# mapbox/robosat

Hardware: AMD Instinct MI355X
Metric: 512x512 tiles/sec train+predict, 1/2/4/8 MI355X; mIoU vs CPU ref (higher is better)
Workload: dtype f32; 1 GPU; rs predict ResNet50-UNet, bs=16 3x512x512 fp32 per GPU, 2 classes (BASELINE configs[1]); parallelism=tiles sharded over 1 rank(s), no collective

## Files before the change

### include/robosat_hip.h

```cpp
#ifndef ROBOSAT_HIP_H
#define ROBOSAT_HIP_H

#include <stdint.h>

#ifdef __cplusplus
extern "C" {
#endif

#define RS_EINVAL (-22)

typedef void* rs_stream_t;

typedef uint16_t rs_bf16;
#define RS_F32 0
#define RS_BF16 1

int rs_abi_version(void);

typedef struct rs_conv_desc {
  int32_t N;
  int32_t Hs, Ws;
  int32_t C1, C2;
  int32_t ups;
  int32_t kh, kw, stride, pad;
// ... 180 lines not shown
int rs_pack_s2_dgrad_phase_weight_dt(const float* w_krsc, void* out, int dtype, int Cout, int Cin, rs_stream_t stream);
int rs_conv2d_fwd_phase_dt(const rs_conv_desc* d, int dtype, const void* src1, const void* src2, const void* weight_phase,
                           const float* scale, const float* shift, const void* residual, const void* relu_mask, void* out,
                           rs_stream_t stream);

int rs_conv2d_splitk(const rs_conv_desc* d, int form, int* rowb);
int rs_conv2d_fwd_splitk(const rs_conv_desc* d, int form, const float* src1, const float* src2, const float* weight,
                         const float* scale, const float* shift, const float* residual, float* out, float* ws, int splits,
                         rs_stream_t stream);

int rs_conv2d_phase_wino_ok(const rs_conv_desc* d);
const char* rs_conv2d_phase_wino_name(const rs_conv_desc* d);
int rs_pack_wino_phase_weight(const float* w_phase, float* u, int Cout, int Cin, rs_stream_t stream);
int rs_conv2d_fwd_phase_wino(const rs_conv_desc* d, const float* src1, const float* src2, const float* u, float* out,
                             rs_stream_t stream);
int rs_conv2d_dgrad_phase_wino_ok(const rs_conv_desc* d);
const char* rs_conv2d_dgrad_phase_wino_name(const rs_conv_desc* d);
int rs_pack_wino_dgrad_weight(const float* wd4x4, float* u, int Cin, int Cout, rs_stream_t stream);
int rs_conv2d_dgrad_phase_wino(const rs_conv_desc* d, const float* dz, const float* u, float* out, const float* mask, float* out2,
                               const float* mask2, int csplit, rs_stream_t stream);

int rs_conv2d_wino33_ok(const rs_conv_desc* d);
const char* rs_conv2d_wino33_name(const rs_conv_desc* d);
int rs_pack_wino33_weight(const float* w_krsc, float* u, int Cout, int Cin, rs_stream_t stream);
int rs_conv2d_fwd_wino33(const rs_conv_desc* d, const float* src, const float* u, const float* scale, const float* shift, float* out,
                         rs_stream_t stream);
int rs_conv2d_wino33_head_ok(const rs_conv_desc* d, int C);
const char* rs_conv2d_wino33_head_name(void);
int rs_conv2d_fwd_wino33_head(const rs_conv_desc* d, const float* src, const float* u, const float* scale, const float* shift,
                              const float* final_w, const float* final_b, int C, int mode, const double* anchors, int overlap,
// ... 170 lines not shown
```

### robosat_amd/_lib.py

```python

import ctypes
import os
from ctypes import POINTER, c_char_p, c_float, c_int, c_int32, c_long, c_void_p

import torch

_HERE = os.path.dirname(os.path.abspath(__file__))
LIB_PATH = os.environ.get("ROBOSAT_HIP_LIB") or os.path.join(_HERE, "librobosat_hip.so")

RS_EINVAL = -22
ABI_VERSION = 24
RS_F32, RS_BF16 = 0, 1
RS_TTA_IN_U8, RS_TTA_IN_F32 = 0, 1
RS_TTA_PROBS, RS_TTA_QUANTIZE, RS_TTA_ARGMAX = 0, 1, 2


class ConvDesc(ctypes.Structure):

    _fields_ = [
        ("N", c_int32), ("Hs", c_int32), ("Ws", c_int32), ("C1", c_int32), ("C2", c_int32), ("ups", c_int32),
        ("kh", c_int32), ("kw", c_int32), ("stride", c_int32), ("pad", c_int32), ("Ho", c_int32), ("Wo", c_int32),
        ("Cout", c_int32), ("relu", c_int32), ("stem", c_int32),
    ]

# ... 78 lines not shown
    "rs_bn_bwd_dt": (c_int, [P, P, P, P, P, P, P, P, P, P, c_int, c_long, c_int, P, P]),
    "rs_upsample2x_bwd_dt": (c_int, [P, P, P, P, P, c_int, c_int, c_int, c_int, c_int, c_int, c_int, P]),
    "rs_conv2d_bnstats_rows": (c_long, [POINTER(ConvDesc)]),
    "rs_conv2d_bnstats_rows_dt": (c_long, [POINTER(ConvDesc), c_int]),
    "rs_conv2d_fwd_bnstats_dt": (c_int, [POINTER(ConvDesc), c_int, P, P, P, P, P, P]),
    "rs_bn_finalize_stats": (c_int, [P, c_long, c_long, c_int, c_float, c_float, P, P, P, P, P, P, P, P, P, P, P]),
    "rs_pack_phase_weight_dt": (c_int, [P, P, c_int, c_int, c_int, P]),
    "rs_pack_s2_dgrad_phase_weight_dt": (c_int, [P, P, c_int, c_int, c_int, P]),
    "rs_conv2d_fwd_phase_dt": (c_int, [POINTER(ConvDesc), c_int, P, P, P, P, P, P, P, P, P]),
    "rs_conv2d_splitk": (c_int, [POINTER(ConvDesc), c_int, POINTER(c_int)]),
    "rs_conv2d_fwd_splitk": (c_int, [POINTER(ConvDesc), c_int, P, P, P, P, P, P, P, P, c_int, P]),
    "rs_conv2d_phase_wino_ok": (c_int, [POINTER(ConvDesc)]),
    "rs_conv2d_phase_wino_name": (c_char_p, [POINTER(ConvDesc)]),
    "rs_pack_wino_phase_weight": (c_int, [P, P, c_int, c_int, P]),
    "rs_conv2d_fwd_phase_wino": (c_int, [POINTER(ConvDesc), P, P, P, P, P]),
    "rs_conv2d_dgrad_phase_wino_ok": (c_int, [POINTER(ConvDesc)]),
    "rs_conv2d_dgrad_phase_wino_name": (c_char_p, [POINTER(ConvDesc)]),
    "rs_pack_wino_dgrad_weight": (c_int, [P, P, c_int, c_int, P]),
    "rs_conv2d_dgrad_phase_wino": (c_int, [POINTER(ConvDesc), P, P, P, P, P, P, c_int, P]),
    "rs_conv2d_wino33_ok": (c_int, [POINTER(ConvDesc)]),
    "rs_conv2d_wino33_name": (c_char_p, [POINTER(ConvDesc)]),
    "rs_pack_wino33_weight": (c_int, [P, P, c_int, c_int, P]),
    "rs_conv2d_fwd_wino33": (c_int, [POINTER(ConvDesc), P, P, P, P, P, P]),
    "rs_conv2d_wino33_head_ok": (c_int, [POINTER(ConvDesc), c_int]),
    "rs_conv2d_wino33_head_name": (c_char_p, []),
    "rs_conv2d_fwd_wino33_head": (c_int, [POINTER(ConvDesc), P, P, P, P, P, P, c_int, c_int, P, c_int, P, P, P]),
    "rs_bottleneck_tail_f32": (c_int, [P, P, P, P, P, P, P, P, P, P, c_long, c_int, c_int, c_int, P]),
    "rs_conv1x1_wave_f32": (c_int, [P, P, P, P, P, c_int, P, c_long, c_int, c_int, P]),
    "rs_conv2d_wino33_stats_rows": (c_long, [POINTER(ConvDesc)]),
    "rs_conv2d_fwd_wino33_stats": (c_int, [POINTER(ConvDesc), P, P, P, P, P]),
# ... 107 lines not shown
```

### robosat_amd/csrc/common.h

```cpp
#pragma once
#include <hip/hip_runtime.h>
#include <stdint.h>

#include "../../include/robosat_hip.h"

typedef float f32x4 __attribute__((ext_vector_type(4)));
typedef float f32x16 __attribute__((ext_vector_type(16)));
typedef __bf16 bf16_t;
typedef __bf16 bf16x4 __attribute__((ext_vector_type(4)));
typedef __bf16 bf16x8 __attribute__((ext_vector_type(8)));
typedef unsigned int u32x2 __attribute__((ext_vector_type(2)));
typedef unsigned int u32x4 __attribute__((ext_vector_type(4)));
typedef short s16x4 __attribute__((ext_vector_type(4)));
typedef short s16x8 __attribute__((ext_vector_type(8)));

__device__ __forceinline__ f32x4 rs_ld4(const float* p) { return *reinterpret_cast<const f32x4*>(p); }
__device__ __forceinline__ f32x4 rs_ld4(const bf16_t* p) {
  return __builtin_convertvector(*reinterpret_cast<const bf16x4*>(p), f32x4);
}
__device__ __forceinline__ void rs_st4(float* p, f32x4 v) { *reinterpret_cast<f32x4*>(p) = v; }
__device__ __forceinline__ void rs_st4(bf16_t* p, f32x4 v) {
  *reinterpret_cast<bf16x4*>(p) = __builtin_convertvector(v, bf16x4);
}
__device__ __forceinline__ float rs_ld1(const float* p) { return *p; }
// ... 166 lines not shown
  int halo_ko = 0;
  int wgrad_f32_phase = 1;
  int wgrad_f32_dma = -1;
  int wgrad_f32_blocks = 2048;
  int wgrad_f32_wino = 1;
  int wgrad_f32_wino_blocks = 1024;
  int wgrad_f32_wino33 = 1;
  int wgrad_f32_wino33_blocks = 256;
  int wgrad_blocks = 96;
  int wgrad_blocks_phase = 1536;
  int wgrad_phase4 = 1;
  int wgrad_blocks_phase4 = 256;
  int wgrad_ring = 3;
  int lovasz_xcd = 1;
  int wino_wide = 1;
  int grow_fused = 0;
};
__attribute__((visibility("hidden"))) RsKnobs& rs_knobs();

__attribute__((visibility("hidden"))) int rs_wgrad_thin_plan(const rs_conv_desc* d, int* blocks, int* slices);
__attribute__((visibility("hidden"))) int rs_wgrad_thin_launch(const rs_conv_desc* d, const void* dy, const void* src,
                                                               float* partial, void* stream);

__attribute__((visibility("hidden"))) int rs_conv_thin_bf16_launch(int mode, const void* src, const void* wgt, const void* mask,
                                                                   void* out, int N, int Hs, int Ws, int relu, void* stream);

__attribute__((visibility("hidden"))) long rs_reduce_scratch_floats(long n, int splits);
__attribute__((visibility("hidden"))) int rs_reduce_splits(const float* ws, float* out, long n, int splits, float* scratch,
                                                           void* stream);

// ... 6 lines not shown
```

### robosat_amd/csrc/conv_wino_f32.hip

```cpp
#define RS_CONV_INSTANTIATE
#include "conv_igemm_dma_kernel.h"

namespace {

struct WinoArgs {
  const float* src1;
  const float* src2;
  const float* u;
  float* out;
  int N, Hs, Ws, C1, C2, Cout;
  int TY, TX;
  int BBY, BBX;
  int nsub;
  int ncb;
  int relu;
  float* out2;
  const float* mask1;
  const float* mask2;
  int csplit;
};

template <int PB>
struct WinoGeom {
  static constexpr int HW = 2 * PB + 1;
  static constexpr int PITCH = HW;
  static constexpr int HALF = PB + 1;
  static constexpr int SBROWS = (HW * PITCH + 7) / 8 * 8;
};

template <int PB>
__device__ __forceinline__ int wino_lane_tile(int l) {
  if constexpr (PB == 8) return ((l & 1) << 1) | (((l >> 1) & 1) << 2) | ((l >> 2) & 1) | (l & 8);
  return ((l & 1) << 1) | (((l >> 1) & 1) << 3) | ((l >> 2) & 1) | (((l >> 3) & 1) << 2);
}
typedef float f32x2 __attribute__((ext_vector_type(2)));
__device__ __forceinline__ f32x2 pk_sub(f32x2 a, f32x2 b) {
  f32x2 d;
  asm("v_pk_add_f32 %0, %1, %2 neg_lo:[0,1] neg_hi:[0,1]" : "=v"(d) : "v"(a), "v"(b));
  return d;
}
__device__ __forceinline__ int wino_lane_now() {
  int l;
  asm volatile("v_mbcnt_lo_u32_b32 %0, -1, 0\n\tv_mbcnt_hi_u32_b32 %0, -1, %0" : "=v"(l));
  return l;
}
__device__ __forceinline__ int wino_swz(int row) { return (row ^ (row >> 1)) & 3; }

template <int PB, int TG, int CG, int NM = 2, bool DG = false>
__global__ __launch_bounds__(512, 1) void conv_wino_f32_kernel(const WinoArgs p) {
  using G = WinoGeom<PB>;
  constexpr int NW = TG * CG;
  static_assert(NW == 8, "8 waves");
  constexpr int BMT = 16 * TG, BN = 16 * NM * CG;
  constexpr int SB = BMT / (PB * PB);
  static_assert(SB * PB * PB == BMT, "whole sub-blocks per block");
  constexpr int AROWS = SB * G::SBROWS;
  constexpr int IA = (AROWS + 15) / 16, IB = 9 * BN / 16;
  constexpr int AROWS_PAD = IA * 16;
  constexpr int JA = (IA + NW - 1) / NW, JB = (IB + NW - 1) / NW;
  constexpr int NI = JA + JB;
  constexpr int STAGE = (AROWS_PAD + 9 * BN) * 64;
  constexpr int KC = 16;

  constexpr int NTR = (AROWS_PAD + 64 * NW - 1) / (64 * NW);
  __shared__ __attribute__((aligned(16))) unsigned char smem[2 * STAGE + 2 * AROWS_PAD * 4 + NTR * 64 * NW * 4];
  int* tabs = reinterpret_cast<int*>(smem + 2 * STAGE);

  int* trows = tabs + 2 * AROWS_PAD;
  const int tid = threadIdx.x, lane = tid & 63;
  const int wave = __builtin_amdgcn_readfirstlane(tid >> 6);
  const int tg = wave % TG, cg = wave / TG;
  const int per_img = p.BBY * p.BBX;
  const int Cin = p.C1 + p.C2;
  const int nk = Cin / KC;
  const int ntiles = ((p.nsub + SB - 1) / SB) * p.ncb * (DG ? 1 : 4);
  const int first = rs_xcd_remap(blockIdx.x, gridDim.x);
  const int nitems = (ntiles - first + (int)gridDim.x - 1) / (int)gridDim.x * (DG ? 4 : 1);
  const unsigned int lds0 = __builtin_amdgcn_readfirstlane(rs_lds_addr(smem));
  const long img1 = (long)p.Hs * p.Ws * p.C1 * (DG ? 4 : 1), img2 = (long)p.Hs * p.Ws * p.C2;

  constexpr int SBS = SB <= 2 ? SB : 1;
  struct Item {
    int py, px, nblk, nfirst, sub0;
    int n[SBS], y0[SBS], x0[SBS];
    bool live[SBS];
  };
  const int uni_first = __builtin_amdgcn_readfirstlane(first), uni_grid = __builtin_amdgcn_readfirstlane((int)gridDim.x);
  const int d_step = DG ? uni_grid : uni_grid >> 2, d_parstep = DG ? 1 : uni_grid & 3;
  int d_par = DG ? 0 : uni_first & 3;
  int d_mblk = (DG ? uni_first : uni_first >> 2) / p.ncb, d_nblk = (DG ? uni_first : uni_first >> 2) - d_mblk * p.ncb;
  const int dq = d_step / p.ncb, dr = d_step - dq * p.ncb;
  auto decode_next = [&](Item& s) __attribute__((always_inline)) {
    s.py = d_par >> 1;
    s.px = d_par & 1;
    if (!DG || d_par == 0) {
      s.nblk = d_nblk;
      const int sub0 = s.sub0 = d_mblk * SB;
      int n = __builtin_amdgcn_readfirstlane(sub0 / per_img);
      const int r2 = sub0 - n * per_img;
      int bby = __builtin_amdgcn_readfirstlane(r2 / p.BBX);
      int bbx = r2 - bby * p.BBX;
      s.nfirst = n;
#pragma unroll
      for (int sb = 0; sb < SBS; ++sb) {
        s.live[sb] = sub0 + sb < p.nsub;
        s.n[sb] = n;
        s.y0[sb] = 2 * bby * PB - 1;
        s.x0[sb] = 2 * bbx * PB - 1;
        if (++bbx == p.BBX) {
          bbx = 0;
          if (++bby == p.BBY) {
            bby = 0;
            ++n;
          }
        }
      }
    }
    d_par += d_parstep;
    const int carry = d_par >> 2;
    d_par &= 3;
    if (!DG || carry) {
      d_mblk += dq;
      d_nblk += dr + (DG ? 0 : carry);
      if (d_nblk >= p.ncb) {
        d_nblk -= p.ncb;
        ++d_mblk;
      }
    }
  };
  Item cur, nxt;
  decode_next(cur);
  nxt = cur;
  auto sub_block = [&](const Item& s, int sb, int& n, int& y0, int& x0, bool& live) __attribute__((always_inline)) {
    if constexpr (SB <= 2) {
      const bool one = SB > 1 && sb > 0;
      n = one ? s.n[SBS - 1] : s.n[0];
      y0 = one ? s.y0[SBS - 1] : s.y0[0];
      x0 = one ? s.x0[SBS - 1] : s.x0[0];
// ... 1 lines not shown
    } else {
      const int sub = s.sub0 + sb;
      n = sub / per_img;
      const int r2 = sub - n * per_img, bby = r2 / p.BBX, bbx = r2 - bby * p.BBX;
      y0 = 2 * bby * PB - 1;
      x0 = 2 * bbx * PB - 1;
      live = sub < p.nsub;
    }
  };

#pragma unroll
  for (int e = 0; e < NTR; ++e) {
    const int rho = tid + 64 * NW * e;
    const int sb = rho / G::SBROWS, rem = rho - sb * G::SBROWS;
    const int hy = rem / G::PITCH, xs = rem - hy * G::PITCH;
    const int hx = xs < G::HALF ? 2 * xs : 2 * (xs - G::HALF) + 1;
    trows[rho] = ((rho < AROWS && hy < G::HW) ? hy << 16 : -(1 << 28)) | (hx << 8) | sb;
  }
  auto build_table = [&](const Item& s, int seq) __attribute__((always_inline)) {
    int* tab = tabs + (seq & 1) * AROWS_PAD;
    const int tnow = 64 * wave + wino_lane_now();
#pragma unroll
    for (int e = 0; e < NTR; ++e) {
      const int rho = tnow + 64 * NW * e;
      if (rho < AROWS_PAD) {
        int n, y0, x0;
        bool live;
        const int row = trows[rho];
        sub_block(s, row & 255, n, y0, x0, live);
        const int y = y0 + s.py + (row >> 16), x = x0 + s.px + ((row >> 8) & 255);
        const bool in = live && (unsigned)y < (unsigned)p.Hs && (unsigned)x < (unsigned)p.Ws;
        const int v = DG ? ((n - s.nfirst) * 2 * p.Hs + 2 * y + 1 - s.py) * (2 * p.Ws) + 2 * x + 1 - s.px
                         : ((n - s.nfirst) * p.Hs + y) * p.Ws + x;
        tab[rho] = in ? v : -1;
      }
    }
    rs_lds_writes_done();
  };

  const int ra = lane >> 2, pp = lane & 3;
  static_assert(128 % BN == 0, "a wave's filter pieces: the same cout, whole positions apart");
  int doff[JA], doffu;
  {
    const int w = 16 * wave + ra, xi = w / BN, co = w - xi * BN;
    doffu = ((xi * p.Cout + co) * Cin) * 4 + ((pp ^ wino_swz(w)) & 3) * 16;
  }
  const int ustep = (128 / BN) * p.Cout * Cin * 4;
  int f_seq = 0, f_kc = 0, f_g = 0;
  int f_nb = 0, f_nfirst = 0;
  __amdgpu_buffer_rsrc_t rsrcs = rs_dma_rsrc<kDmaClamp>(p.src1, 0), rsrcu = rsrcs;
  auto fetch_item = [&](const Item& s) __attribute__((always_inline)) {
    f_nfirst = s.nfirst;
    f_nb = s.nblk * BN * Cin * 4;
    rsrcu = rs_dma_rsrc<kDmaClamp>(p.u + (long)(2 * s.py + s.px) * 9 * p.Cout * Cin, (long)9 * p.Cout * Cin * 4);
  };
  auto set_source = [&](bool src_first) __attribute__((always_inline)) {
    const int cb = (src_first ? p.C1 : p.C2) * 4;
    rsrcs = rs_dma_rsrc<kDmaClamp>(src_first ? p.src1 + f_nfirst * img1 : p.src2 + f_nfirst * img2,
                                   (long)(p.N - f_nfirst) * (src_first ? img1 : img2) * 4);
    const int* tab = tabs + (f_seq & 1) * AROWS_PAD;
    int pix[JA];
#pragma unroll
    for (int j = 0; j < JA; ++j) {
      const int ii = wave + NW * j;
      pix[j] = tab[16 * (ii < IA ? ii : IA - 1) + ra];
    }
#pragma unroll
    for (int j = 0; j < JA; ++j) {
      const int ii = wave + NW * j;
// ... 4 lines not shown
  auto fetch_chunk = [&](auto interleave, bool past) __attribute__((always_inline)) {
    const int c0 = f_kc * KC;
    const bool src_first = c0 < p.C1;
    if (!past) {
      if (f_kc == 0) fetch_item(nxt);
      if (c0 == 0 || c0 == p.C1) set_source(src_first);
    }
    const unsigned int fL = lds0 + (f_g & 1) * STAGE;
    const int fsa = __builtin_amdgcn_readfirstlane((src_first ? c0 : c0 - p.C1) * 4), fsu = __builtin_amdgcn_readfirstlane(c0 * 4 + f_nb);
    interleave([&](int j) __attribute__((always_inline)) {
      if (j < JA) {
        const int ii = wave + NW * j;
        if (j < JA - 1 || JA * NW == IA || ii < IA) rs_dma16(rsrcs, fL + ii * 1024, doff[j], fsa);
      } else {
        const int fi = wave + NW * (j - JA);
        if (j < NI - 1 || JB * NW == IB || fi < IB) rs_dma16(rsrcu, fL + (IA + fi) * 1024, doffu, fsu + (j - JA) * ustep);
      }
    });
    ++f_g;
    if (!past && ++f_kc == nk) {
      f_kc = 0;
      ++f_seq;
    }
  };

  const int l15 = lane & 15, pc = lane >> 4;
  const int t = 16 * tg + wino_lane_tile<PB>(l15);
  const int tsb = 16 * tg / (PB * PB), tq = t - tsb * (PB * PB);
  const int tty = tq / PB, ttx = tq - tty * PB;
  int addrA[3][3];
  {
    const int rho0 = tsb * G::SBROWS + 2 * tty * G::PITCH + ttx;
#pragma unroll
    for (int r = 0; r < 3; ++r)
#pragma unroll
      for (int c = 0; c < 3; ++c) {
        const int rho = rho0 + r * G::PITCH + (c == 0 ? 0 : (c == 1 ? G::HALF : 1));
        addrA[r][c] = rho * 64 + ((pc ^ wino_swz(rho)) & 3) * 16;
      }
  }
  const int addrB = AROWS_PAD * 64 + (16 * NM * cg + l15) * 64 + ((pc ^ wino_swz(l15)) & 3) * 16;

  build_table(cur, 0);
  __syncthreads();
  fetch_chunk([&](auto issue) __attribute__((always_inline)) {
#pragma unroll
    for (int j = 0; j < NI; ++j) issue(j);
  }, false);
  const int total = nitems * nk;
  const int Ho = 2 * p.Hs, Wo = 2 * p.Ws;

#ifdef RS_WINO_TAIL2
  constexpr int TAIL = NM >= 4 ? 1 : RS_WINO_TAIL2;
#else
  constexpr int TAIL = NM >= 4 ? 1 : PB == 4 ? 2 : (DG || TG == 8) ? 0 : 1;
#endif
  static_assert(TAIL >= 0 && TAIL <= 2, "positions behind the barrier");
  constexpr int NMMA = 36 * NM, NHEAD = (9 - TAIL) * 4 * NM, NT = TAIL * 4 * NM;
  constexpr int PSTEP = 2 * NMMA / 3 / NI >= 1 ? 2 * NMMA / 3 / NI : 1;
  static_assert((NI - 1) * PSTEP < NHEAD, "the DMA pieces go out in the chunk's head");
  f32x4 V[9], Bq[9][NM];
  auto chunk_head = [&](const unsigned char* L, f32x4(&Vn)[9], f32x4(&B0)[NM], auto tail, auto nt) __attribute__((always_inline)) {
    constexpr int N = decltype(nt)::value, LEAD = N / 2;
    f32x4 P[3][3];
#pragma unroll
    for (int r = 0; r < 3; ++r)
#pragma unroll
      for (int c = 0; c < 3; ++c) P[r][c] = *reinterpret_cast<const f32x4*>(L + addrA[r][c]);
    __builtin_amdgcn_sched_barrier(0);
#pragma unroll
// ... 106 lines not shown
            const int a = a0 + u, b = b0 + v;
            if (a >= p.Hs || b >= p.Ws) continue;
            const long o = ((long)(e_n * p.Hs + a) * p.Ws + b) * ostride + ocol;
#pragma unroll
            for (int m = 0; m < NM; ++m) {
              f32x4 y = (acc[u * 3 + v][m] + acc[u * 3 + v + 1][m]) + (acc[(u + 1) * 3 + v][m] + acc[(u + 1) * 3 + v + 1][m]);
              if (mb) {
                const f32x4 z = *reinterpret_cast<const f32x4*>(mb + o + 16 * m);
#pragma unroll
                for (int e = 0; e < 4; ++e) y[e] = z[e] > 0.f ? y[e] : 0.f;
              }
              *reinterpret_cast<f32x4*>(ob + o + 16 * m) = y;
            }
          }
      }
    } else if (e_live) {
      float* obase = p.out + cur.nblk * BN + 16 * NM * cg + 4 * e_pc;
#pragma unroll
      for (int u = 0; u < 2; ++u)
#pragma unroll
        for (int v = 0; v < 2; ++v) {
          const int a = a0 + u, b = b0 + v;
          if (a >= p.Hs || b >= p.Ws) continue;
          float* o = obase + ((long)(e_n * Ho + 2 * a + cur.py) * Wo + 2 * b + cur.px) * p.Cout;
#pragma unroll
          for (int m = 0; m < NM; ++m) {
            f32x4 y = (acc[u * 3 + v][m] + acc[u * 3 + v + 1][m]) + (acc[(u + 1) * 3 + v][m] + acc[(u + 1) * 3 + v + 1][m]);
            if (p.relu) {
#pragma unroll
              for (int e = 0; e < 4; ++e) y[e] = fmaxf(y[e], 0.f);
// ... 26 lines not shown
  const int co = (int)(i % Cout);
  const long r = i / Cout;
  const int ci = (int)(r % Cin), ph = (int)(r / Cin), py = ph >> 1, px = ph & 1;
  const float* g = wd + (long)ci * 16 * Cout + co;
  const float g00 = g[(long)(py * 4 + px) * Cout], g01 = g[(long)(py * 4 + 2 + px) * Cout];
  const float g10 = g[(long)((2 + py) * 4 + px) * Cout], g11 = g[(long)((2 + py) * 4 + 2 + px) * Cout];
  const float v[9] = {g00, g00 + g01, g01, g00 + g10, (g00 + g01) + (g10 + g11), g01 + g11, g10, g10 + g11, g11};
#pragma unroll
  for (int x = 0; x < 9; ++x) u[(((long)ph * 9 + x) * Cin + ci) * Cout + co] = v[x];
}

bool wino_wide() {
  return rs_knobs().wino_wide != 0;
}

struct WinoPlan {
  int pb, wgn;
  int sb;
  bool worth;
  bool wide;
};

bool wino_plan(const rs_conv_desc* d, WinoPlan* pl) {
  if (!d || d->N <= 0 || d->Hs <= 0 || d->Ws <= 0 || d->C1 <= 0 || (d->C1 % 16) || d->C2 < 0 || (d->C2 % 16) || d->Cout <= 0 ||
      (d->Cout % 32))
    return false;
  if (!(d->ups == 1 && d->kh == 3 && d->kw == 3 && d->stride == 1 && d->pad == 1 && d->Ho == 2 * d->Hs && d->Wo == 2 * d->Ws)) return false;
  const int ty = (d->Hs + 1) / 2, tx = (d->Ws + 1) / 2;
  if (ty < 4 || tx < 4) return false;
  pl->pb = (ty >= 8 && tx >= 8) ? 8 : 4;
  pl->wgn = (d->Cout % 64 == 0) ? 2 : 1;
  pl->sb = 16 * (8 / pl->wgn) / (pl->pb * pl->pb);
  if (d->C1 + d->C2 < 32) return false;
  const long cmax = d->C1 > d->C2 ? d->C1 : d->C2;
  if ((long)(pl->sb + 1) * d->Hs * d->Ws * cmax * 4 >= (1L << 31)) return false;
  if ((long)9 * d->Cout * (d->C1 + d->C2) * 4 >= (1L << 31)) return false;
  if ((long)d->N * d->Ho * d->Wo >= (1L << 31)) return false;
  pl->worth = pl->pb == 8;
  pl->wide = false;
  if (pl->pb == 8 && pl->wgn == 2 && wino_wide()) {
    const long nsub = (long)d->N * rs_cdiv(ty, 8) * rs_cdiv(tx, 8);
    pl->wide = (nsub + 1) / 2 * (d->Cout / 64) * 4 >= 2L * rs_cu_count();
    if (pl->wide) pl->sb = 2;
  }
  return true;
}

}

extern "C" int rs_conv2d_phase_wino_ok(const rs_conv_desc* d) {
  WinoPlan pl;
  if (!wino_plan(d, &pl)) return 0;
  return pl.worth ? 1 : 2;
}

extern "C" const char* rs_conv2d_phase_wino_name(const rs_conv_desc* d) {
  WinoPlan pl;
  if (!wino_plan(d, &pl)) return "";
  if (pl.pb == 8) return pl.wide ? "conv_wino_f32<phase,p8,128x64>" : (pl.wgn == 2 ? "conv_wino_f32<phase,p8,64x64>" : "conv_wino_f32<phase,p8,128x32>");
  return pl.wgn == 2 ? "conv_wino_f32<phase,p4,64x64>" : "conv_wino_f32<phase,p4,128x32>";
}

extern "C" int rs_pack_wino_phase_weight(const float* w_phase, float* u, int Cout, int Cin, rs_stream_t stream) {
  if (!w_phase || !u || Cout <= 0 || Cin <= 0) return RS_EINVAL;
  const long total = 4L * Cout * Cin;
  pack_wino_phase_weight_kernel<<<rs_cdiv(total, 256), 256, 0, (hipStream_t)stream>>>(w_phase, u, Cout, Cin, total);
  return RS_LAUNCH_RESULT();
}

extern "C" int rs_conv2d_fwd_phase_wino(const rs_conv_desc* d, const float* src1, const float* src2, const float* u, float* out,
                                        rs_stream_t stream) {
  WinoPlan pl;
  if (!wino_plan(d, &pl) || !src1 || !u || !out || (d->C2 > 0 && !src2)) return RS_EINVAL;
  WinoArgs a;
  a.src1 = src1;
  a.src2 = src2;
  a.u = u;
  a.out = out;
  a.N = d->N;
  a.Hs = d->Hs;
  a.Ws = d->Ws;
  a.C1 = d->C1;
  a.C2 = d->C2;
  a.Cout = d->Cout;
  a.TY = (d->Hs + 1) / 2;
  a.TX = (d->Ws + 1) / 2;
  a.BBY = rs_cdiv(a.TY, pl.pb);
  a.BBX = rs_cdiv(a.TX, pl.pb);
  a.nsub = d->N * a.BBY * a.BBX;
  a.ncb = d->Cout / (32 * pl.wgn);
  a.relu = d->relu;
  a.out2 = nullptr;
  a.mask1 = a.mask2 = nullptr;
  a.csplit = 0;
  const long items = (long)rs_cdiv(a.nsub, pl.sb) * a.ncb * 4;
  if (items >= (1L << 31)) return RS_EINVAL;
  const int grid = (int)(items < rs_cu_count() ? items : rs_cu_count());
  hipStream_t s = (hipStream_t)stream;
  if (pl.wide) conv_wino_f32_kernel<8, 8, 1, 4><<<grid, 512, 0, s>>>(a);
  else if (pl.pb == 8 && pl.wgn == 2) conv_wino_f32_kernel<8, 4, 2><<<grid, 512, 0, s>>>(a);
  else if (pl.pb == 8) conv_wino_f32_kernel<8, 8, 1><<<grid, 512, 0, s>>>(a);
  else if (pl.wgn == 2) conv_wino_f32_kernel<4, 4, 2><<<grid, 512, 0, s>>>(a);
  else conv_wino_f32_kernel<4, 8, 1><<<grid, 512, 0, s>>>(a);
  return RS_LAUNCH_RESULT();
}

namespace {
bool wino_dgrad_plan(const rs_conv_desc* d, rs_conv_desc* g, WinoPlan* pl) {
  if (!d || d->C1 <= 0 || d->C2 < 0 || d->Cout <= 0) return false;
  *g = *d;
  g->C1 = d->Cout;
  g->C2 = 0;
  g->Cout = d->C1 + d->C2;
  if (!wino_plan(g, pl) || !pl->worth) return false;
  if ((long)(pl->sb + 1) * 4 * d->Hs * d->Ws * g->C1 * 4 >= (1L << 31)) return false;
  if (g->Cout % 64) return false;
  return true;
}
}

extern "C" int rs_conv2d_dgrad_phase_wino_ok(const rs_conv_desc* d) {
  rs_conv_desc g;
  WinoPlan pl;
  return wino_dgrad_plan(d, &g, &pl) ? 1 : 0;
}

extern "C" const char* rs_conv2d_dgrad_phase_wino_name(const rs_conv_desc* d) {
  rs_conv_desc g;
  WinoPlan pl;
  if (!wino_dgrad_plan(d, &g, &pl)) return "";
  return pl.wide ? "conv_wino_f32<dgrad4x4,p8,128x64>" : "conv_wino_f32<dgrad4x4,p8,64x64>";
// ... 22 lines not shown
  a.mask2 = mask2;
  a.csplit = csplit;
  a.N = d->N;
  a.Hs = d->Hs;
  a.Ws = d->Ws;
  a.C1 = g.C1;
  a.C2 = 0;
  a.Cout = g.Cout;
  a.TY = (d->Hs + 1) / 2;
  a.TX = (d->Ws + 1) / 2;
  a.BBY = rs_cdiv(a.TY, pl.pb);
  a.BBX = rs_cdiv(a.TX, pl.pb);
  a.nsub = d->N * a.BBY * a.BBX;
  a.ncb = g.Cout / 64;
  a.relu = 0;
  bool wide = false;
  if (wino_wide()) wide = (long)((a.nsub + 1) / 2) * a.ncb >= 2L * rs_cu_count();
  const int sb = wide ? 2 : 1;
  const long items = (long)rs_cdiv(a.nsub, sb) * a.ncb;
  if (items >= (1L << 29)) return RS_EINVAL;
  const int grid = (int)(items < rs_cu_count() ? items : rs_cu_count());
  hipStream_t s = (hipStream_t)stream;
  if (wide) conv_wino_f32_kernel<8, 8, 1, 4, true><<<grid, 512, 0, s>>>(a);
  else conv_wino_f32_kernel<8, 4, 2, 2, true><<<grid, 512, 0, s>>>(a);
  return RS_LAUNCH_RESULT();
}
```

### robosat_amd/csrc/knobs.hip

```cpp
#include <stdio.h>
#include <stdlib.h>
#include <string.h>

#include "common.h"

namespace {

struct Entry {
  const char* name;
  const char* env;
  int RsKnobs::*field;
  int lo, hi;
};

bool in_range(const Entry& e, int v) {
  if (v < e.lo || v > e.hi) return false;
  if (e.field == &RsKnobs::conv_rowb) return v == 0 || v == 64 || v == 128;
  return true;
}

const Entry kEntries[] = {
    {"conv_tile", "RS_CONV_TILE", &RsKnobs::conv_tile, -1, 9},
    {"conv_rowb", "RS_CONV_ROWB", &RsKnobs::conv_rowb, 0, 128},
    {"conv_big", "RS_CONV_BIG", &RsKnobs::conv_big, 0, 1},
// ... 8 lines not shown
    {"halo_ko", "RS_HALO_KO", &RsKnobs::halo_ko, 0, 4},
    {"wgrad_f32_phase", "RS_WGRAD_F32_PHASE", &RsKnobs::wgrad_f32_phase, 0, 1},
    {"wgrad_f32_dma", "RS_WGRAD_F32_DMA", &RsKnobs::wgrad_f32_dma, -1, 1},
    {"wgrad_f32_blocks", "RS_WGRAD_F32_BLOCKS", &RsKnobs::wgrad_f32_blocks, 1, 1048576},
    {"wgrad_f32_wino", "RS_WGRAD_F32_WINO", &RsKnobs::wgrad_f32_wino, 0, 1},
    {"wgrad_f32_wino_blocks", "RS_WGRAD_F32_WINO_BLOCKS", &RsKnobs::wgrad_f32_wino_blocks, 1, 1048576},
    {"wgrad_f32_wino33", "RS_WGRAD_F32_WINO33", &RsKnobs::wgrad_f32_wino33, 0, 1},
    {"wgrad_f32_wino33_blocks", "RS_WGRAD_F32_WINO33_BLOCKS", &RsKnobs::wgrad_f32_wino33_blocks, 1, 1048576},
    {"wgrad_blocks", "RS_WGRAD_BLOCKS", &RsKnobs::wgrad_blocks, 1, 1048576},
    {"wgrad_blocks_phase", "RS_WGRAD_BLOCKS_PHASE", &RsKnobs::wgrad_blocks_phase, 1, 1048576},
    {"wgrad_phase4", "RS_WGRAD_PHASE4", &RsKnobs::wgrad_phase4, 0, 1},
    {"wgrad_blocks_phase4", "RS_WGRAD_BLOCKS_PHASE4", &RsKnobs::wgrad_blocks_phase4, 1, 1048576},
    {"wgrad_ring", "RS_WGRAD_RING", &RsKnobs::wgrad_ring, 2, 7},
    {"lovasz_xcd", "RS_LOVASZ_XCD", &RsKnobs::lovasz_xcd, 0, 1},
    {"wino_wide", "ROBOSAT_WINO_WIDE", &RsKnobs::wino_wide, 0, 1},
    {"grow_fused", "RS_GROW_FUSED", &RsKnobs::grow_fused, 0, 16},
};

}

RsKnobs& rs_knobs() {
  static RsKnobs k = [] {
    RsKnobs v;
    for (const Entry& e : kEntries)
      if (const char* s = getenv(e.env)) {
        const int x = atoi(s);
        if (in_range(e, x)) v.*(e.field) = x;
        else fprintf(stderr, "robosat_hip: %s=%s is outside [%d, %d]: ignored, the rule stays\n", e.env, s, e.lo, e.hi);
      }
    return v;
// ... 25 lines not shown
```

### robosat_amd/ops.py

```python

import ctypes
import os

import torch

from . import _lib
from ._lib import RS_BF16, RS_F32, ConvDesc, check

BF16 = torch.bfloat16


def _dt(t):

    dtype = getattr(t, "dtype", t)
    if dtype == torch.float32:
        return RS_F32
    if dtype == torch.bfloat16:
        return RS_BF16
    raise TypeError("robosat_amd: activations are fp32 or bf16, got {}".format(dtype))


def _esize(t):

    return 2 if getattr(t, "dtype", t) == BF16 else 4
# ... 338 lines not shown
    if src1.dtype != torch.float32 or not (force or switch("ROBOSAT_WINOGRAD")):
        return False
    d = _phase_desc(*src1.shape, 0 if src2 is None else src2.shape[3], cout)
    rc = _lib.lib().rs_conv2d_phase_wino_ok(ctypes.byref(d))
    return rc != 0 if force else rc == 1


def pack_wino_phase_weight(weight_phase):

    _, cout, _, _, cin = weight_phase.shape
    u = torch.empty((4, 9, cout, cin), device=weight_phase.device, dtype=torch.float32)
    _call("rs_pack_wino_phase_weight", _dev(weight_phase, "w_phase"), _dev(u, "u"), cout, cin, _stream())
    return u


def conv2d_phase_wino(src1, u, src2=None, relu=False):

    n, hs, ws, c1 = src1.shape
    c2 = 0 if src2 is None else src2.shape[3]
    cout = u.shape[2]
    assert tuple(u.shape) == (4, 9, cout, c1 + c2)
    if src2 is not None and tuple(src2.shape[:3]) != (n, hs, ws):
        raise RuntimeError("Sizes of tensors must match except in dimension 1: skip {} vs decoder {}".format(
            tuple(src1.shape[:3]), tuple(src2.shape[:3])))
    d = _phase_desc(n, hs, ws, c1, c2, cout, relu)
    out = torch.empty((n, 2 * hs, 2 * ws, cout), device=src1.device, dtype=torch.float32)
    ev = _start()
    _call("rs_conv2d_fwd_phase_wino", ctypes.byref(d), _dev(src1, "src1"), _dev(src2, "src2"), _dev(u, "u"), _dev(out, "out"), _stream())
    if ev:
        _stop(ev)
        name = _lib.lib().rs_conv2d_phase_wino_name(ctypes.byref(d)).decode()
        _record(ev, name, conv_flops(d), _shape(d), conv_bytes(d, 4), conv_flops(d) * 0.25)
    return out


def wino_dgrad_ok(n, hs, ws, c1, c2, cout):

    if not switch("ROBOSAT_WINO_DGRAD"):
        return False
    return _lib.lib().rs_conv2d_dgrad_phase_wino_ok(ctypes.byref(_phase_desc(n, hs, ws, c1, c2, cout))) == 1


def pack_wino_dgrad_weight(wd4x4):
# ... 1709 lines not shown
```

### robosat_amd/unet.py

```python

import math
import os
import warnings

import torch
import torch.nn as nn

from . import ops

_RESNET50_FILE = "resnet50-19c8e357.pth"


class _Conv(nn.Module):

    def __init__(self, cin, cout, k, stride=1, padding=0, bias=False, init="default"):
        super().__init__()
        self.cin, self.cout, self.k, self.stride, self.padding = cin, cout, k, stride, padding
        w = torch.empty(cout, cin, k, k).contiguous(memory_format=torch.channels_last)
        fan_in, fan_out = cin * k * k, cout * k * k
        if init == "resnet":
            nn.init.normal_(w, 0.0, math.sqrt(2.0 / fan_out))
        else:
            nn.init.uniform_(w, -1.0 / math.sqrt(fan_in), 1.0 / math.sqrt(fan_in))
        self.weight = nn.Parameter(w)
# ... 176 lines not shown
    def __init__(self, num_in, num_out):
        super().__init__()
        self.block = ConvRelu(num_in, num_out)


def conv3x3_eval(conv, x, dt, scale=None, shift=None):

    if dt == torch.float32 and conv.stride == 1 and ops.wino33_ok(x, conv.cout):
        return ops.conv2d_wino33(x, conv.wino33(), scale=scale, shift=shift, relu=True)
    return ops.conv2d(x, conv.krsc(dt), stride=conv.stride, pad=1, scale=scale, shift=shift, relu=True)


def decoder_block(conv, skip, prev, dt):

    if dt == torch.float32 and ops.wino_ok(skip, prev, conv.cout):
        return ops.conv2d_phase_wino(skip, conv.phase_wino(), src2=prev, relu=True)
    return ops.conv2d_phase(skip, conv.phase(dt), src2=prev, relu=True)


def _find_pretrained():
    cands = [os.environ.get("ROBOSAT_RESNET50_WEIGHTS")]
    home = os.environ.get("TORCH_HOME", os.path.join(os.path.expanduser("~"), ".cache", "torch"))
    cands += [os.path.join(home, "checkpoints", _RESNET50_FILE), os.path.join(home, "hub", "checkpoints", _RESNET50_FILE)]
    for c in cands:
        if c and os.path.isfile(c):
            return c
    return None


class UNet(nn.Module):

# ... 317 lines not shown
```

Baseline: 1729 tiles/s.

## Add pixel-form Winograd for upsampled decoder convs computing all four phases per tile

Adds a PIX variant of the Winograd forward kernel for the decoder's upsample+3x3 conv. Each block now loads a 10x10 source-pixel halo and computes all four output phases from shared 3x3 products on the low-resolution grid, combining adjacent accumulators in the epilogue. This replaces the four separate per-phase passes over the input, removing repeated input loads and transforms and a quarter of the item count. The trade-off is a different weight indexing (per-position offsets into the 36-slot phase weights), extra epilogue adds, and no tail-behind-barrier overlap. It is enabled by default through decoder_block and a new knob.

```diff
diff --git a/include/robosat_hip.h b/include/robosat_hip.h
--- a/include/robosat_hip.h
+++ b/include/robosat_hip.h
@@ -218,6 +218,8 @@
 int rs_pack_wino_phase_weight(const float* w_phase, float* u, int Cout, int Cin, rs_stream_t stream);
 int rs_conv2d_fwd_phase_wino(const rs_conv_desc* d, const float* src1, const float* src2, const float* u, float* out,
                              rs_stream_t stream);
+int rs_conv2d_fwd_upsampled_wino(const rs_conv_desc* d, const float* src1, const float* src2, const float* u, float* out,
+                                 rs_stream_t stream);
 int rs_conv2d_dgrad_phase_wino_ok(const rs_conv_desc* d);
 const char* rs_conv2d_dgrad_phase_wino_name(const rs_conv_desc* d);
 int rs_pack_wino_dgrad_weight(const float* wd4x4, float* u, int Cin, int Cout, rs_stream_t stream);
diff --git a/robosat_amd/_lib.py b/robosat_amd/_lib.py
--- a/robosat_amd/_lib.py
+++ b/robosat_amd/_lib.py
@@ -116,6 +116,7 @@
     "rs_conv2d_phase_wino_name": (c_char_p, [POINTER(ConvDesc)]),
     "rs_pack_wino_phase_weight": (c_int, [P, P, c_int, c_int, P]),
     "rs_conv2d_fwd_phase_wino": (c_int, [POINTER(ConvDesc), P, P, P, P, P]),
+    "rs_conv2d_fwd_upsampled_wino": (c_int, [POINTER(ConvDesc), P, P, P, P, P]),
     "rs_conv2d_dgrad_phase_wino_ok": (c_int, [POINTER(ConvDesc)]),
     "rs_conv2d_dgrad_phase_wino_name": (c_char_p, [POINTER(ConvDesc)]),
     "rs_pack_wino_dgrad_weight": (c_int, [P, P, c_int, c_int, P]),
diff --git a/robosat_amd/csrc/common.h b/robosat_amd/csrc/common.h
--- a/robosat_amd/csrc/common.h
+++ b/robosat_amd/csrc/common.h
@@ -204,6 +204,7 @@
   int wgrad_ring = 3;
   int lovasz_xcd = 1;
   int wino_wide = 1;
+  int wino_pixel = 1;
   int grow_fused = 0;
 };
 __attribute__((visibility("hidden"))) RsKnobs& rs_knobs();
diff --git a/robosat_amd/csrc/conv_wino_f32.hip b/robosat_amd/csrc/conv_wino_f32.hip
--- a/robosat_amd/csrc/conv_wino_f32.hip
+++ b/robosat_amd/csrc/conv_wino_f32.hip
@@ -20,9 +20,9 @@
   int csplit;
 };
 
-template <int PB>
+template <int PB, bool PIX = false>
 struct WinoGeom {
-  static constexpr int HW = 2 * PB + 1;
+  static constexpr int HW = PIX ? 10 : 2 * PB + 1;
   static constexpr int PITCH = HW;
   static constexpr int HALF = PB + 1;
   static constexpr int SBROWS = (HW * PITCH + 7) / 8 * 8;
@@ -33,6 +33,8 @@
   if constexpr (PB == 8) return ((l & 1) << 1) | (((l >> 1) & 1) << 2) | ((l >> 2) & 1) | (l & 8);
   return ((l & 1) << 1) | (((l >> 1) & 1) << 3) | ((l >> 2) & 1) | (((l >> 3) & 1) << 2);
 }
+__device__ __forceinline__ int wino_lane_pixel_y(int l) { return l & 3; }
+__device__ __forceinline__ int wino_lane_pixel_x(int l) { return (l >> 2) & 3; }
 typedef float f32x2 __attribute__((ext_vector_type(2)));
 __device__ __forceinline__ f32x2 pk_sub(f32x2 a, f32x2 b) {
   f32x2 d;
@@ -46,11 +48,13 @@
 }
 __device__ __forceinline__ int wino_swz(int row) { return (row ^ (row >> 1)) & 3; }
 
-template <int PB, int TG, int CG, int NM = 2, bool DG = false>
+template <int PB, int TG, int CG, int NM = 2, bool DG = false, bool PIX = false>
 __global__ __launch_bounds__(512, 1) void conv_wino_f32_kernel(const WinoArgs p) {
-  using G = WinoGeom<PB>;
+  using G = WinoGeom<PB, PIX>;
   constexpr int NW = TG * CG;
   static_assert(NW == 8, "8 waves");
+  static_assert(!PIX || (PB == 8 && !DG), "the pixel form: forward, 64-row sub-blocks");
+  constexpr bool PAR = !DG && !PIX;
   constexpr int BMT = 16 * TG, BN = 16 * NM * CG;
   constexpr int SB = BMT / (PB * PB);
   static_assert(SB * PB * PB == BMT, "whole sub-blocks per block");
@@ -73,7 +77,7 @@
   const int per_img = p.BBY * p.BBX;
   const int Cin = p.C1 + p.C2;
   const int nk = Cin / KC;
-  const int ntiles = ((p.nsub + SB - 1) / SB) * p.ncb * (DG ? 1 : 4);
+  const int ntiles = ((p.nsub + SB - 1) / SB) * p.ncb * (PAR ? 4 : 1);
   const int first = rs_xcd_remap(blockIdx.x, gridDim.x);
   const int nitems = (ntiles - first + (int)gridDim.x - 1) / (int)gridDim.x * (DG ? 4 : 1);
   const unsigned int lds0 = __builtin_amdgcn_readfirstlane(rs_lds_addr(smem));
@@ -86,13 +90,13 @@
     bool live[SBS];
   };
   const int uni_first = __builtin_amdgcn_readfirstlane(first), uni_grid = __builtin_amdgcn_readfirstlane((int)gridDim.x);
-  const int d_step = DG ? uni_grid : uni_grid >> 2, d_parstep = DG ? 1 : uni_grid & 3;
-  int d_par = DG ? 0 : uni_first & 3;
-  int d_mblk = (DG ? uni_first : uni_first >> 2) / p.ncb, d_nblk = (DG ? uni_first : uni_first >> 2) - d_mblk * p.ncb;
+  const int d_step = PAR ? uni_grid >> 2 : uni_grid, d_parstep = DG ? 1 : uni_grid & 3;
+  int d_par = PAR ? uni_first & 3 : 0;
+  int d_mblk = (PAR ? uni_first >> 2 : uni_first) / p.ncb, d_nblk = (PAR ? uni_first >> 2 : uni_first) - d_mblk * p.ncb;
   const int dq = d_step / p.ncb, dr = d_step - dq * p.ncb;
   auto decode_next = [&](Item& s) __attribute__((always_inline)) {
-    s.py = d_par >> 1;
-    s.px = d_par & 1;
+    s.py = PIX ? 0 : d_par >> 1;
+    s.px = PIX ? 0 : d_par & 1;
     if (!DG || d_par == 0) {
       s.nblk = d_nblk;
       const int sub0 = s.sub0 = d_mblk * SB;
@@ -105,8 +109,8 @@
       for (int sb = 0; sb < SBS; ++sb) {
         s.live[sb] = sub0 + sb < p.nsub;
         s.n[sb] = n;
-        s.y0[sb] = 2 * bby * PB - 1;
-        s.x0[sb] = 2 * bbx * PB - 1;
+        s.y0[sb] = (PIX ? 8 : 2 * PB) * bby - 1;
+        s.x0[sb] = (PIX ? 8 : 2 * PB) * bbx - 1;
         if (++bbx == p.BBX) {
           bbx = 0;
           if (++bby == p.BBY) {
@@ -116,12 +120,15 @@
         }
       }
     }
-    d_par += d_parstep;
-    const int carry = d_par >> 2;
-    d_par &= 3;
+    int carry = 0;
+    if constexpr (!PIX) {
+      d_par += d_parstep;
+      carry = d_par >> 2;
+      d_par &= 3;
+    }
     if (!DG || carry) {
       d_mblk += dq;
-      d_nblk += dr + (DG ? 0 : carry);
+      d_nblk += dr + (PAR ? carry : 0);
       if (d_nblk >= p.ncb) {
         d_nblk -= p.ncb;
         ++d_mblk;
@@ -153,7 +160,7 @@
     const int rho = tid + 64 * NW * e;
     const int sb = rho / G::SBROWS, rem = rho - sb * G::SBROWS;
     const int hy = rem / G::PITCH, xs = rem - hy * G::PITCH;
-    const int hx = xs < G::HALF ? 2 * xs : 2 * (xs - G::HALF) + 1;
+    const int hx = PIX ? xs : xs < G::HALF ? 2 * xs : 2 * (xs - G::HALF) + 1;
     trows[rho] = ((rho < AROWS && hy < G::HW) ? hy << 16 : -(1 << 28)) | (hx << 8) | sb;
   }
   auto build_table = [&](const Item& s, int seq) __attribute__((always_inline)) {
@@ -167,7 +174,7 @@
         bool live;
         const int row = trows[rho];
         sub_block(s, row & 255, n, y0, x0, live);
-        const int y = y0 + s.py + (row >> 16), x = x0 + s.px + ((row >> 8) & 255);
+        const int y = y0 + (PIX ? 0 : s.py) + (row >> 16), x = x0 + (PIX ? 0 : s.px) + ((row >> 8) & 255);
         const bool in = live && (unsigned)y < (unsigned)p.Hs && (unsigned)x < (unsigned)p.Ws;
         const int v = DG ? ((n - s.nfirst) * 2 * p.Hs + 2 * y + 1 - s.py) * (2 * p.Ws) + 2 * x + 1 - s.px
                          : ((n - s.nfirst) * p.Hs + y) * p.Ws + x;
@@ -179,19 +186,25 @@
 
   const int ra = lane >> 2, pp = lane & 3;
   static_assert(128 % BN == 0, "a wave's filter pieces: the same cout, whole positions apart");
-  int doff[JA], doffu;
+  int doff[JA], doffu, upos[JB];
   {
-    const int w = 16 * wave + ra, xi = w / BN, co = w - xi * BN;
+    const int w = 16 * wave + ra, xi = PIX ? 0 : w / BN, co = w - (w / BN) * BN;
     doffu = ((xi * p.Cout + co) * Cin) * 4 + ((pp ^ wino_swz(w)) & 3) * 16;
   }
   const int ustep = (128 / BN) * p.Cout * Cin * 4;
+#pragma unroll
+  for (int j = 0; j < JB; ++j) {
+    const int fi = wave + NW * j, xi = fi < IB ? 16 * fi / BN : 8, r = xi / 3, c = xi - 3 * r;
+    upos[j] = PIX ? __builtin_amdgcn_readfirstlane(((2 * (r == 2) + (c == 2)) * 9 + xi) * p.Cout * Cin * 4) : 0;
+  }
   int f_seq = 0, f_kc = 0, f_g = 0;
   int f_nb = 0, f_nfirst = 0;
-  __amdgpu_buffer_rsrc_t rsrcs = rs_dma_rsrc<kDmaClamp>(p.src1, 0), rsrcu = rsrcs;
+  __amdgpu_buffer_rsrc_t rsrcs = rs_dma_rsrc<kDmaClamp>(p.src1, 0);
+  __amdgpu_buffer_rsrc_t rsrcu = PIX ? rs_dma_rsrc<kDmaClamp>(p.u, (long)36 * p.Cout * Cin * 4) : rsrcs;
   auto fetch_item = [&](const Item& s) __attribute__((always_inline)) {
     f_nfirst = s.nfirst;
     f_nb = s.nblk * BN * Cin * 4;
-    rsrcu = rs_dma_rsrc<kDmaClamp>(p.u + (long)(2 * s.py + s.px) * 9 * p.Cout * Cin, (long)9 * p.Cout * Cin * 4);
+    if constexpr (!PIX) rsrcu = rs_dma_rsrc<kDmaClamp>(p.u + (long)(2 * s.py + s.px) * 9 * p.Cout * Cin, (long)9 * p.Cout * Cin * 4);
   };
   auto set_source = [&](bool src_first) __attribute__((always_inline)) {
     const int cb = (src_first ? p.C1 : p.C2) * 4;
@@ -226,7 +239,7 @@
         if (j < JA - 1 || JA * NW == IA || ii < IA) rs_dma16(rsrcs, fL + ii * 1024, doff[j], fsa);
       } else {
         const int fi = wave + NW * (j - JA);
-        if (j < NI - 1 || JB * NW == IB || fi < IB) rs_dma16(rsrcu, fL + (IA + fi) * 1024, doffu, fsu + (j - JA) * ustep);
+        if (j < NI - 1 || JB * NW == IB || fi < IB) rs_dma16(rsrcu, fL + (IA + fi) * 1024, doffu, fsu + (PIX ? upos[j - JA] : (j - JA) * ustep));
       }
     });
     ++f_g;
@@ -240,14 +253,16 @@
   const int t = 16 * tg + wino_lane_tile<PB>(l15);
   const int tsb = 16 * tg / (PB * PB), tq = t - tsb * (PB * PB);
   const int tty = tq / PB, ttx = tq - tty * PB;
+  const int wby = (tg >> 1) & 1, wbx = tg & 1;
   int addrA[3][3];
   {
-    const int rho0 = tsb * G::SBROWS + 2 * tty * G::PITCH + ttx;
+    const int rho0 = PIX ? tsb * G::SBROWS + (4 * wby + wino_lane_pixel_y(l15)) * G::PITCH + 4 * wbx + wino_lane_pixel_x(l15)
+                         : tsb * G::SBROWS + 2 * tty * G::PITCH + ttx;
 #pragma unroll
     for (int r = 0; r < 3; ++r)
 #pragma unroll
       for (int c = 0; c < 3; ++c) {
-        const int rho = rho0 + r * G::PITCH + (c == 0 ? 0 : (c == 1 ? G::HALF : 1));
+        const int rho = rho0 + r * G::PITCH + (PIX ? c : c == 0 ? 0 : (c == 1 ? G::HALF : 1));
         addrA[r][c] = rho * 64 + ((pc ^ wino_swz(rho)) & 3) * 16;
       }
   }
@@ -262,10 +277,16 @@
   const int total = nitems * nk;
   const int Ho = 2 * p.Hs, Wo = 2 * p.Ws;
 
-#ifdef RS_WINO_TAIL2
-  constexpr int TAIL = NM >= 4 ? 1 : RS_WINO_TAIL2;
+#if defined(RS_WINO_TAIL2) || defined(RS_WINO_TAIL4)
+#ifndef RS_WINO_TAIL2
+#define RS_WINO_TAIL2 (PIX ? 0 : PB == 4 ? 2 : (DG || TG == 8) ? 0 : 1)
+#endif
+#ifndef RS_WINO_TAIL4
+#define RS_WINO_TAIL4 (PIX ? 0 : 1)
+#endif
+  constexpr int TAIL = NM >= 4 ? RS_WINO_TAIL4 : RS_WINO_TAIL2;
 #else
-  constexpr int TAIL = NM >= 4 ? 1 : PB == 4 ? 2 : (DG || TG == 8) ? 0 : 1;
+  constexpr int TAIL = PIX ? 0 : NM >= 4 ? 1 : PB == 4 ? 2 : (DG || TG == 8) ? 0 : 1;
 #endif
   static_assert(TAIL >= 0 && TAIL <= 2, "positions behind the barrier");
   constexpr int NMMA = 36 * NM, NHEAD = (9 - TAIL) * 4 * NM, NT = TAIL * 4 * NM;
@@ -402,6 +423,26 @@
             }
           }
       }
+    } else if constexpr (PIX) {
+      const int a = e_y0 + 1 + 4 * wby + wino_lane_pixel_y(e_lane & 15), b = e_x0 + 1 + 4 * wbx + wino_lane_pixel_x(e_lane & 15);
+      if (e_live && a < p.Hs && b < p.Ws) {
+        float* obase = p.out + cur.nblk * BN + 16 * NM * cg + 4 * e_pc + ((long)(e_n * Ho + 2 * a) * Wo + 2 * b) * p.Cout;
+#pragma unroll
+        for (int u = 0; u < 2; ++u)
+#pragma unroll
+          for (int v = 0; v < 2; ++v) {
+            float* o = obase + ((long)u * Wo + v) * p.Cout;
+#pragma unroll
+            for (int m = 0; m < NM; ++m) {
+              f32x4 y = (acc[u * 3 + v][m] + acc[u * 3 + v + 1][m]) + (acc[(u + 1) * 3 + v][m] + acc[(u + 1) * 3 + v + 1][m]);
+              if (p.relu) {
+#pragma unroll
+                for (int e = 0; e < 4; ++e) y[e] = fmaxf(y[e], 0.f);
+              }
+              *reinterpret_cast<f32x4*>(o + 16 * m) = y;
+            }
+          }
+      }
     } else if (e_live) {
       float* obase = p.out + cur.nblk * BN + 16 * NM * cg + 4 * e_pc;
 #pragma unroll
@@ -458,14 +499,22 @@
   return rs_knobs().wino_wide != 0;
 }
 
+constexpr bool kWinoPixel64 = true, kWinoPixel32 = true;
+bool wino_pixel(int wgn) { return (wgn == 2 ? kWinoPixel64 : kWinoPixel32) && rs_knobs().wino_pixel != 0; }
+
+bool wino_wide_rule(long regions, int ncb, int units) {
+  return wino_wide() && (regions + 1) / 2 * ncb * units >= 2L * rs_cu_count();
+}
+
 struct WinoPlan {
   int pb, wgn;
   int sb;
+  bool pix;
   bool worth;
   bool wide;
 };
 
-bool wino_plan(const rs_conv_desc* d, WinoPlan* pl) {
+bool wino_plan(const rs_conv_desc* d, WinoPlan* pl, bool fwd = true, bool upsampled = false) {
   if (!d || d->N <= 0 || d->Hs <= 0 || d->Ws <= 0 || d->C1 <= 0 || (d->C1 % 16) || d->C2 < 0 || (d->C2 % 16) || d->Cout <= 0 ||
       (d->Cout % 32))
     return false;
@@ -480,13 +529,10 @@
   if ((long)(pl->sb + 1) * d->Hs * d->Ws * cmax * 4 >= (1L << 31)) return false;
   if ((long)9 * d->Cout * (d->C1 + d->C2) * 4 >= (1L << 31)) return false;
   if ((long)d->N * d->Ho * d->Wo >= (1L << 31)) return false;
+  pl->pix = fwd && upsampled && pl->pb == 8 && wino_pixel(pl->wgn) && (long)4 * 9 * d->Cout * (d->C1 + d->C2) * 4 < (1L << 31);
   pl->worth = pl->pb == 8;
-  pl->wide = false;
-  if (pl->pb == 8 && pl->wgn == 2 && wino_wide()) {
-    const long nsub = (long)d->N * rs_cdiv(ty, 8) * rs_cdiv(tx, 8);
-    pl->wide = (nsub + 1) / 2 * (d->Cout / 64) * 4 >= 2L * rs_cu_count();
-    if (pl->wide) pl->sb = 2;
-  }
+  pl->wide = pl->pb == 8 && pl->wgn == 2 && wino_wide_rule((long)d->N * rs_cdiv(d->Hs, 16) * rs_cdiv(d->Ws, 16), d->Cout / 64, 4);
+  if (pl->wide) pl->sb = 2;
   return true;
 }
 
@@ -512,10 +558,11 @@
   return RS_LAUNCH_RESULT();
 }
 
-extern "C" int rs_conv2d_fwd_phase_wino(const rs_conv_desc* d, const float* src1, const float* src2, const float* u, float* out,
-                                        rs_stream_t stream) {
+namespace {
+int wino_fwd_launch(const rs_conv_desc* d, const float* src1, const float* src2, const float* u, float* out, rs_stream_t stream,
+                    bool upsampled) {
   WinoPlan pl;
-  if (!wino_plan(d, &pl) || !src1 || !u || !out || (d->C2 > 0 && !src2)) return RS_EINVAL;
+  if (!wino_plan(d, &pl, true, upsampled) || !src1 || !u || !out || (d->C2 > 0 && !src2)) return RS_EINVAL;
   WinoArgs a;
   a.src1 = src1;
   a.src2 = src2;
@@ -529,24 +576,39 @@
   a.Cout = d->Cout;
   a.TY = (d->Hs + 1) / 2;
   a.TX = (d->Ws + 1) / 2;
-  a.BBY = rs_cdiv(a.TY, pl.pb);
-  a.BBX = rs_cdiv(a.TX, pl.pb);
+  a.BBY = pl.pix ? rs_cdiv(d->Hs, 8) : rs_cdiv(a.TY, pl.pb);
+  a.BBX = pl.pix ? rs_cdiv(d->Ws, 8) : rs_cdiv(a.TX, pl.pb);
+  if ((long)d->N * a.BBY * a.BBX >= (1L << 31)) return RS_EINVAL;
   a.nsub = d->N * a.BBY * a.BBX;
   a.ncb = d->Cout / (32 * pl.wgn);
   a.relu = d->relu;
   a.out2 = nullptr;
   a.mask1 = a.mask2 = nullptr;
   a.csplit = 0;
-  const long items = (long)rs_cdiv(a.nsub, pl.sb) * a.ncb * 4;
+  const long items = (long)rs_cdiv(a.nsub, pl.sb) * a.ncb * (pl.pix ? 1 : 4);
   if (items >= (1L << 31)) return RS_EINVAL;
   const int grid = (int)(items < rs_cu_count() ? items : rs_cu_count());
   hipStream_t s = (hipStream_t)stream;
-  if (pl.wide) conv_wino_f32_kernel<8, 8, 1, 4><<<grid, 512, 0, s>>>(a);
+  if (pl.pix && pl.wide) conv_wino_f32_kernel<8, 8, 1, 4, false, true><<<grid, 512, 0, s>>>(a);
+  else if (pl.pix && pl.wgn == 2) conv_wino_f32_kernel<8, 4, 2, 2, false, true><<<grid, 512, 0, s>>>(a);
+  else if (pl.pix) conv_wino_f32_kernel<8, 8, 1, 2, false, true><<<grid, 512, 0, s>>>(a);
+  else if (pl.wide) conv_wino_f32_kernel<8, 8, 1, 4><<<grid, 512, 0, s>>>(a);
   else if (pl.pb == 8 && pl.wgn == 2) conv_wino_f32_kernel<8, 4, 2><<<grid, 512, 0, s>>>(a);
   else if (pl.pb == 8) conv_wino_f32_kernel<8, 8, 1><<<grid, 512, 0, s>>>(a);
   else if (pl.wgn == 2) conv_wino_f32_kernel<4, 4, 2><<<grid, 512, 0, s>>>(a);
   else conv_wino_f32_kernel<4, 8, 1><<<grid, 512, 0, s>>>(a);
   return RS_LAUNCH_RESULT();
+}
+}
+
+extern "C" int rs_conv2d_fwd_phase_wino(const rs_conv_desc* d, const float* src1, const float* src2, const float* u, float* out,
+                                        rs_stream_t stream) {
+  return wino_fwd_launch(d, src1, src2, u, out, stream, false);
+}
+
+extern "C" int rs_conv2d_fwd_upsampled_wino(const rs_conv_desc* d, const float* src1, const float* src2, const float* u, float* out,
+                                            rs_stream_t stream) {
+  return wino_fwd_launch(d, src1, src2, u, out, stream, true);
 }
 
 namespace {
@@ -556,9 +618,11 @@
   g->C1 = d->Cout;
   g->C2 = 0;
   g->Cout = d->C1 + d->C2;
-  if (!wino_plan(g, pl) || !pl->worth) return false;
+  if (!wino_plan(g, pl, false) || !pl->worth) return false;
   if ((long)(pl->sb + 1) * 4 * d->Hs * d->Ws * g->C1 * 4 >= (1L << 31)) return false;
   if (g->Cout % 64) return false;
+  pl->wide = wino_wide_rule((long)d->N * rs_cdiv(d->Hs, 16) * rs_cdiv(d->Ws, 16), g->Cout / 64, 1);
+  pl->sb = pl->wide ? 2 : 1;
   return true;
 }
 }
@@ -611,10 +675,8 @@
   a.nsub = d->N * a.BBY * a.BBX;
   a.ncb = g.Cout / 64;
   a.relu = 0;
-  bool wide = false;
-  if (wino_wide()) wide = (long)((a.nsub + 1) / 2) * a.ncb >= 2L * rs_cu_count();
-  const int sb = wide ? 2 : 1;
-  const long items = (long)rs_cdiv(a.nsub, sb) * a.ncb;
+  const bool wide = pl.wide;
+  const long items = (long)rs_cdiv(a.nsub, pl.sb) * a.ncb;
   if (items >= (1L << 29)) return RS_EINVAL;
   const int grid = (int)(items < rs_cu_count() ? items : rs_cu_count());
   hipStream_t s = (hipStream_t)stream;
diff --git a/robosat_amd/csrc/knobs.hip b/robosat_amd/csrc/knobs.hip
--- a/robosat_amd/csrc/knobs.hip
+++ b/robosat_amd/csrc/knobs.hip
@@ -46,6 +46,7 @@
     {"wgrad_ring", "RS_WGRAD_RING", &RsKnobs::wgrad_ring, 2, 7},
     {"lovasz_xcd", "RS_LOVASZ_XCD", &RsKnobs::lovasz_xcd, 0, 1},
     {"wino_wide", "ROBOSAT_WINO_WIDE", &RsKnobs::wino_wide, 0, 1},
+    {"wino_pixel", "ROBOSAT_WINO_PIXEL", &RsKnobs::wino_pixel, 0, 1},
     {"grow_fused", "RS_GROW_FUSED", &RsKnobs::grow_fused, 0, 16},
 };
 
diff --git a/robosat_amd/ops.py b/robosat_amd/ops.py
--- a/robosat_amd/ops.py
+++ b/robosat_amd/ops.py
@@ -376,7 +376,7 @@
     return u
 
 
-def conv2d_phase_wino(src1, u, src2=None, relu=False):
+def conv2d_phase_wino(src1, u, src2=None, relu=False, upsampled=False):
 
     n, hs, ws, c1 = src1.shape
     c2 = 0 if src2 is None else src2.shape[3]
@@ -388,7 +388,8 @@
     d = _phase_desc(n, hs, ws, c1, c2, cout, relu)
     out = torch.empty((n, 2 * hs, 2 * ws, cout), device=src1.device, dtype=torch.float32)
     ev = _start()
-    _call("rs_conv2d_fwd_phase_wino", ctypes.byref(d), _dev(src1, "src1"), _dev(src2, "src2"), _dev(u, "u"), _dev(out, "out"), _stream())
+    _call("rs_conv2d_fwd_upsampled_wino" if upsampled else "rs_conv2d_fwd_phase_wino", ctypes.byref(d),
+          _dev(src1, "src1"), _dev(src2, "src2"), _dev(u, "u"), _dev(out, "out"), _stream())
     if ev:
         _stop(ev)
         name = _lib.lib().rs_conv2d_phase_wino_name(ctypes.byref(d)).decode()
diff --git a/robosat_amd/unet.py b/robosat_amd/unet.py
--- a/robosat_amd/unet.py
+++ b/robosat_amd/unet.py
@@ -214,7 +214,7 @@
 def decoder_block(conv, skip, prev, dt):
 
     if dt == torch.float32 and ops.wino_ok(skip, prev, conv.cout):
-        return ops.conv2d_phase_wino(skip, conv.phase_wino(), src2=prev, relu=True)
+        return ops.conv2d_phase_wino(skip, conv.phase_wino(), src2=prev, relu=True, upsampled=True)
     return ops.conv2d_phase(skip, conv.phase(dt), src2=prev, relu=True)
 
 
```

New measurement: 1754 tiles/s, median of 6. 1.01x the previous value.
